# qfall/tools

Measured on AMD Instinct MI355X. Metric: preimages/sec (whole node) + HBM-BW% for samp_p, n=512 q~2^30 batch=4096, higher is better.
Workload: dtype f64+int64

## Files before the change

tools_amd/csrc/psf_kernels.hpp:

```cpp
#pragma once
#include <hip/hip_runtime.h>
#include <cstdint>
#include "psf_rng.hpp"

namespace psf {

typedef double d4 __attribute__((ext_vector_type(4)));
typedef int v4i __attribute__((ext_vector_type(4)));
typedef __attribute__((address_space(3))) void* lds_void_ptr;

constexpr int TR_BM = 128;
constexpr int TR_BN = 128;
#ifndef PSF_TR_BK
#define PSF_TR_BK 16
#endif
constexpr int TR_BK = PSF_TR_BK;
constexpr int TR_CHUNK = TR_BM * TR_BK;
constexpr int TR_KB_PER_BLOCK = TR_BM / TR_BK;

__host__ __device__ inline size_t tr_rowblock_base(size_t bi) { return (size_t)TR_KB_PER_BLOCK * bi * (bi + 1) / 2; }
__host__ __device__ inline size_t tr_total_chunks(size_t nbi) { return (size_t)TR_KB_PER_BLOCK * nbi * (nbi + 1) / 2; }

__host__ __device__ inline int tr_chunk_pos(int r, int kk) {
  return ((kk >> 2) * 8 + (r >> 4)) * 64 + ((kk & 3) << 4) + (r & 15);
}

template <bool PACKED>
__global__ void k_repack_L(const double* __restrict__ src, size_t ld, size_t m, double* __restrict__ dst, size_t nbi) {
  const size_t total = tr_total_chunks(nbi) * TR_CHUNK;
  for (size_t g = (size_t)blockIdx.x * blockDim.x + threadIdx.x; g < total; g += (size_t)gridDim.x * blockDim.x) {
    const size_t chunk = g / TR_CHUNK;
    const int pos = (int)(g % TR_CHUNK);
    size_t bi = (size_t)((sqrt(1.0 + 8.0 * (double)chunk / TR_KB_PER_BLOCK) - 1.0) * 0.5);
    while (tr_rowblock_base(bi + 1) <= chunk) ++bi;
    while (tr_rowblock_base(bi) > chunk) --bi;
    const size_t bk = chunk - tr_rowblock_base(bi);
    const int ks = pos >> 9, tile = (pos >> 6) & 7, lane = pos & 63;
    const size_t row = bi * TR_BM + tile * 16 + (lane & 15);
    const size_t col = bk * TR_BK + ks * 4 + (lane >> 4);
    double v = 0.0;
    if (row < m && col <= row) v = PACKED ? src[row * (row + 1) / 2 + col] : src[row * ld + col];
    dst[g] = v;
  }
}

__global__ void k_unpack_L(const double* __restrict__ chunks, size_t first, size_t total, double* __restrict__ packed) {
  for (size_t g0 = (size_t)blockIdx.x * blockDim.x + threadIdx.x; g0 < total; g0 += (size_t)gridDim.x * blockDim.x) {
    const size_t g = first + g0;
    size_t row = (size_t)((sqrt(1.0 + 8.0 * (double)g) - 1.0) * 0.5);
    while ((row + 1) * (row + 2) / 2 <= g) ++row;
    while (row * (row + 1) / 2 > g) --row;
    const size_t col = g - row * (row + 1) / 2;
    const size_t bi = row / TR_BM, bk = col / TR_BK;
    const size_t chunk = tr_rowblock_base(bi) + bk;
    packed[g0] = chunks[chunk * TR_CHUNK + tr_chunk_pos((int)(row % TR_BM), (int)(col % TR_BK))];
  }
}

constexpr int NR_SEG = 4096;
__host__ inline uint32_t nr_segment(size_t total) {
  size_t seg = (total / 4096 + 63) / 64 * 64;
  if (seg < 128) seg = 128;
  return (uint32_t)(seg > (size_t)NR_SEG ? (size_t)NR_SEG : seg);
}
__device__ inline int lane_rank(uint64_t mask);
__host__ __device__ inline uint32_t udiv_magic_of(uint32_t d) { return d < 2 ? 0u : (uint32_t)((((uint64_t)1 << 32) + d - 1) / d); }
__device__ inline void udivmod_magic(uint32_t o, uint32_t d, uint32_t M, uint32_t* q, uint32_t* r) {
  const uint32_t qq = M ? __umulhi(o, M) : o;
  *q = qq;
  *r = o - qq * d;
}

struct NormalsFixed { size_t split; int8_t* planes; size_t plane_bytes; size_t ld; double* X; double h; };
constexpr int kFixPlanes = 5;

__global__ __launch_bounds__(256) void k_normals_wave(uint64_t seed, uint64_t first_index, size_t m, size_t B, size_t nkb, size_t nbj,
                                                      double* __restrict__ Dt, int* __restrict__ fail, NormalsFixed fx, uint32_t ncf, uint32_t seg) {
  const int lane = threadIdx.x & 63;
  const size_t total = ncf >= 0x100u ? nkb * 4 * 4 * (size_t)(ncf - 0x100u) : ncf ? nkb * 4 * (size_t)ncf * 64 : nbj * nkb * TR_CHUNK;
  const size_t seg0 = ((size_t)blockIdx.x * 4 + (threadIdx.x >> 6)) * seg;
  if (seg0 >= total) return;
  const size_t seg1 = seg0 + seg < total ? seg0 + seg : total;
  const size_t chunk0 = seg0 / TR_CHUNK;
  constexpr int NCH = NR_SEG / TR_CHUNK + 1;
  size_t cbj[NCH], cbk[NCH];
// ... 41 lines not shown
        const uint64_t index = first_index + b;
        const U4 w = philox(seed, (uint32_t)coord, (uint32_t)index, t, tag_word(TAG_NORMAL, index));
        const double u = (double)(((((uint64_t)w.y << 32) | w.x) >> 11) + 1) * 0x1.0p-53;
        const uint64_t vv = (((uint64_t)w.w << 32) | w.z) >> 12;
        const double x = (((double)(2 * vv + 1) * 0x1.0p-52 - 1.0) * 0.8577638849607068) / u;
        {
          const float xf = (float)x, uf = (float)u;
          const float e32 = __builtin_amdgcn_exp2f(-0.36067376f * (xf * xf));
          const bool sure = uf <= e32 * 0.9998f, never = uf > e32 * 1.0002f;
          accept = sure;
          if (!sure && !never) accept = u <= det_exp(-0.25 * (x * x));
        }
        v = x;
        if (!accept && ++t >= kMaxAttempts) { accept = true; f = 1; v = 0.0; }
        if (accept && fx.planes && coord >= fx.split) {
          const double sc = floor(v * 0x1.0p32 + 0.5);
          if (!(fabs(sc) < 0x1.0p38)) f = 1;
          long long qv = (long long)sc;
          v = sc * 0x1.0p-32;
          const size_t c = coord - fx.split;
          const size_t addr = ((c >> 4) * fx.ld + b) * 16 + (c & 15);
#pragma unroll
          for (int pl = 0; pl < kFixPlanes; ++pl) {
            const long long dg = (long long)(int8_t)(qv & 0xff);
            fx.planes[(size_t)pl * fx.plane_bytes + addr] = (int8_t)dg;
            qv = (qv - dg) >> 8;
          }
          fx.X[coord * fx.ld + b] = fx.h * v;
        }
      }
      if (accept) Dt[my] = v;
    }
    const uint64_t mask = __ballot(accept);
    if (mask) {
      const size_t nid = next_free + (size_t)lane_rank(mask);
      if (accept) {
        my = nid;
        active = nid < seg1;
        t = 0;
        if (active) locate(nid, &coord, &b);
      }
      next_free += (size_t)__popcll(mask);
    }
  }
  if (f) atomicOr(fail, 1);
}

__global__ __launch_bounds__(256) void k_narrow_rows(const int64_t* __restrict__ src, int32_t* __restrict__ dst, size_t count, int* __restrict__ overflow) {
  const size_t stride = (size_t)gridDim.x * 256;
  int bad = 0;
  const size_t pairs = count / 2;
  for (size_t i = (size_t)blockIdx.x * 256 + threadIdx.x; i < pairs; i += stride) {
    const longlong2 v = reinterpret_cast<const longlong2*>(src)[i];
    bad |= (v.x != (int64_t)(int32_t)v.x) | (v.y != (int64_t)(int32_t)v.y);
    reinterpret_cast<int2*>(dst)[i] = make_int2((int32_t)v.x, (int32_t)v.y);
  }
  if ((count & 1) && blockIdx.x == 0 && threadIdx.x == 0) {
    const int64_t v = src[count - 1];
    bad |= v != (int64_t)(int32_t)v;
    dst[count - 1] = (int32_t)v;
  }
  if (bad) atomicOr(overflow, 1);
}

__global__ __launch_bounds__(256) void k_copy_words(const uint64_t* __restrict__ host_src, uint64_t* __restrict__ dst, size_t count) {
  const size_t stride = (size_t)gridDim.x * 256, pairs = count / 2;
  typedef unsigned long long u2 __attribute__((ext_vector_type(2)));
  for (size_t i = (size_t)blockIdx.x * 256 + threadIdx.x; i < pairs; i += stride)
    reinterpret_cast<u2*>(dst)[i] = __builtin_nontemporal_load(reinterpret_cast<const u2*>(host_src) + i);
  if ((count & 1) && blockIdx.x == 0 && threadIdx.x == 0) dst[count - 1] = host_src[count - 1];
}

__global__ void k_export_normals(const double* __restrict__ Dt, size_t m, size_t B, size_t nkb, double* __restrict__ out , uint32_t ncf) {
  const size_t total = m * B;
  for (size_t g = (size_t)blockIdx.x * blockDim.x + threadIdx.x; g < total; g += (size_t)gridDim.x * blockDim.x) {
    const size_t b = g / m, coord = g % m;
    if (ncf >= 0x100u) { out[g] = Dt[((coord / 4) * (ncf - 0x100u) + b) * 4 + coord % 4]; continue; }
    if (ncf) { out[g] = Dt[((coord / 4) * ncf + b / 16) * 64 + (coord % 4) * 16 + b % 16]; continue; }
    const size_t chunk = (b / TR_BN) * nkb + coord / TR_BK;
    out[g] = Dt[chunk * TR_CHUNK + tr_chunk_pos((int)(b % TR_BN), (int)(coord % TR_BK))];
  }
}

__device__ inline void tr_map_block(unsigned id, int nbi, int nbj, int GR, int GC, int* bi, int* bj) {
  const int ncg = (nbj + GC - 1) / GC, nrg = (nbi + GR - 1) / GR;
  const unsigned xcd = id & 7u, slot = id >> 3;
  const unsigned group = (slot / (GR * GC)) * 8u + xcd;
  const unsigned t = slot % (GR * GC);
  const int rg = nrg - 1 - (int)(group / ncg), cg = (int)(group % ncg);
  *bi = rg * GR + (GR - 1 - (int)(t / GC));
  *bj = cg * GC + (int)(t % GC);
  if (rg < 0) *bi = -1;
}
__host__ inline unsigned tr_grid_size(int nbi, int nbj, int GR = 8, int GC = 8) {
  const int ncg = (nbj + GC - 1) / GC, nrg = (nbi + GR - 1) / GR;
  const unsigned groups = (unsigned)(ncg * nrg);
  const unsigned rounds = (groups + 7) / 8;
  return rounds * 8u * (unsigned)(GR * GC);
}

#ifdef TRMM_CLOCK_PROBE
__device__ unsigned long long g_trmm_clk[4];
__device__ unsigned long long* g_trmm_log;
#define TR_CLK_BEGIN const unsigned long long clk0 = clock64(), rt0 = wall_clock64();
#define TR_CLK_END if (threadIdx.x == 0) { const unsigned long long rt1 = wall_clock64(); atomicAdd(&g_trmm_clk[0], clock64() - clk0); atomicAdd(&g_trmm_clk[1], rt1 - rt0); atomicAdd(&g_trmm_clk[2], 1ull); \
    if (g_trmm_log) { g_trmm_log[2 * (size_t)blockIdx.x] = rt0; g_trmm_log[2 * (size_t)blockIdx.x + 1] = rt1; } }
#else
#define TR_CLK_BEGIN
#define TR_CLK_END
#endif

constexpr int TR_PD = 6;
#define TR_LOAD8(dst, voff, base, imm) asm volatile("global_load_dwordx2 %0, %1, %2 offset:" #imm : "=v"(dst) : "v"(voff), "s"(base) : "memory")
#define TR_WAIT(n, A, Bv) asm volatile("s_waitcnt vmcnt(" #n ")" : "+v"(A[0]), "+v"(A[1]), "+v"(A[2]), "+v"(A[3]), "+v"(Bv[0]), "+v"(Bv[1]), "+v"(Bv[2]), "+v"(Bv[3]))

constexpr int TR_BIG_PD = 4;
#ifndef TR_BIG_UNROLL
#define TR_BIG_UNROLL 2
#endif
#define TR_WAIT12(n, A, Bv) asm volatile("s_waitcnt vmcnt(" #n ")" : "+v"(A[0]), "+v"(A[1]), "+v"(A[2]), "+v"(A[3]), "+v"(A[4]), "+v"(A[5]), "+v"(A[6]), "+v"(A[7]), \
                                         "+v"(Bv[0]), "+v"(Bv[1]), "+v"(Bv[2]), "+v"(Bv[3]))
__global__ __launch_bounds__(256, 1) void k_trmm_f64_big(const double* __restrict__ Lt, const double* __restrict__ Dt,
                                                         double* __restrict__ X, int nbi, int nbj, size_t nkb, size_t ldx, int GR, int GC, size_t row_hi) {
  int bt, bj;
  const int nbt = (nbi + 1) / 2;
  tr_map_block(blockIdx.x, nbt, nbj, GR, GC, &bt, &bj);
  if (bt < 0 || bt >= nbt || bj >= nbj) return;
  TR_CLK_BEGIN
  const int tid = threadIdx.x, lane = tid & 63;
  const int wave = __builtin_amdgcn_readfirstlane(tid >> 6);
  const int wr = wave >> 1, wc = wave & 1;
  const int bi = 2 * bt + wr;
  if (bi < nbi) {
    const int nsteps = TR_KB_PER_BLOCK * (bi + 1) * (TR_BK / 4);
    const double* gA = Lt + tr_rowblock_base((size_t)bi) * TR_CHUNK;
    const double* gB = Dt + (size_t)bj * nkb * TR_CHUNK + (size_t)(wc * 4) * 64;
    const uint32_t voff = (uint32_t)lane * 8u;
    d4 acc[8][4];
#pragma unroll
    for (int i = 0; i < 8; ++i)
#pragma unroll
      for (int j = 0; j < 4; ++j) acc[i][j] = d4{0.0, 0.0, 0.0, 0.0};
    double a[TR_BIG_PD][8], b[TR_BIG_PD][4];
    auto issue = [&](double (&av)[8], double (&bv)[4], int s) {
      const double* pa = gA + (size_t)s * 512;
      const double* pb = gB + (size_t)s * 512;
      TR_LOAD8(av[0], voff, pa, 0); TR_LOAD8(av[1], voff, pa, 512); TR_LOAD8(av[2], voff, pa, 1024); TR_LOAD8(av[3], voff, pa, 1536);
      TR_LOAD8(av[4], voff, pa, 2048); TR_LOAD8(av[5], voff, pa, 2560); TR_LOAD8(av[6], voff, pa, 3072); TR_LOAD8(av[7], voff, pa, 3584);
      TR_LOAD8(bv[0], voff, pb, 0); TR_LOAD8(bv[1], voff, pb, 512); TR_LOAD8(bv[2], voff, pb, 1024); TR_LOAD8(bv[3], voff, pb, 1536);
    };
#define TR_MFMA(i, j) asm volatile("v_mfma_f64_16x16x4_f64 %0, %1, %2, %0" : "+a"(acc[i][j]) : "v"(av[i]), "v"(bv[j]))
    auto step = [&](double (&av)[8], double (&bv)[4], int sn) {
      const double* pa = gA + (size_t)sn * 512;
      const double* pb = gB + (size_t)sn * 512;
      TR_MFMA(0, 0); TR_MFMA(0, 1); TR_MFMA(0, 2); TR_MFMA(0, 3); TR_LOAD8(av[0], voff, pa, 0);
      TR_MFMA(1, 0); TR_MFMA(1, 1); TR_MFMA(1, 2); TR_MFMA(1, 3); TR_LOAD8(av[1], voff, pa, 512);
      TR_MFMA(2, 0); TR_MFMA(2, 1); TR_MFMA(2, 2); TR_MFMA(2, 3); TR_LOAD8(av[2], voff, pa, 1024);
      TR_MFMA(3, 0); TR_MFMA(3, 1); TR_MFMA(3, 2); TR_MFMA(3, 3); TR_LOAD8(av[3], voff, pa, 1536);
      TR_MFMA(4, 0); TR_MFMA(4, 1); TR_MFMA(4, 2); TR_MFMA(4, 3); TR_LOAD8(av[4], voff, pa, 2048);
      TR_MFMA(5, 0); TR_MFMA(5, 1); TR_MFMA(5, 2); TR_MFMA(5, 3); TR_LOAD8(av[5], voff, pa, 2560);
      TR_MFMA(6, 3); TR_MFMA(7, 3); TR_LOAD8(bv[3], voff, pb, 1536);
      TR_MFMA(6, 2); TR_MFMA(7, 2); TR_LOAD8(bv[2], voff, pb, 1024);
      TR_MFMA(6, 1); TR_MFMA(7, 1); TR_LOAD8(bv[1], voff, pb, 512);
      TR_MFMA(6, 0); TR_MFMA(7, 0); TR_LOAD8(bv[0], voff, pb, 0);
      TR_LOAD8(av[6], voff, pa, 3072); TR_LOAD8(av[7], voff, pa, 3584);
    };
#pragma unroll
    for (int u = 0; u < TR_BIG_PD; ++u) issue(a[u], b[u], u);
    for (int s0 = 0; s0 < nsteps; s0 += TR_BIG_PD * TR_BIG_UNROLL) {
#pragma unroll
      for (int rnd = 0; rnd < TR_BIG_UNROLL; ++rnd)
#pragma unroll
      for (int u = 0; u < TR_BIG_PD; ++u) {
        TR_WAIT12(36, a[u], b[u]);
        static_assert(TR_BIG_PD == 4, "the wait count above is 12 (TR_BIG_PD - 1)");
        int sn = s0 + rnd * TR_BIG_PD + u + TR_BIG_PD;
        sn = sn < nsteps ? sn : nsteps - 1;
        step(a[u], b[u], sn);
      }
    }
#undef TR_MFMA
#pragma unroll
    for (int u = 0; u < TR_BIG_PD; ++u) TR_WAIT12(0, a[u], b[u]);
    asm volatile("s_nop 15\n\ts_nop 15\n\ts_nop 15\n\ts_nop 15\n\ts_nop 15" ::: "memory");
    const size_t row0 = (size_t)bi * TR_BM, col0 = (size_t)bj * TR_BN + wc * 64;
#pragma unroll
    for (int i = 0; i < 8; ++i)
#pragma unroll
      for (int j = 0; j < 4; ++j)
#pragma unroll
        for (int r = 0; r < 4; ++r)
        {
          const size_t row = row0 + i * 16 + (lane >> 4) + 4 * r;
          if (row < row_hi) X[row * ldx + col0 + j * 16 + (lane & 15)] = acc[i][j][r];
        }
  }
  TR_CLK_END
}

constexpr int PR_SEG = 4096;
constexpr long long kDigitRangeP = (1ll << 23) - 1;

__device__ inline double wave_xor_sum(double x) {
  typedef unsigned int u2v __attribute__((ext_vector_type(2)));
  auto mk = [](uint32_t lo, uint32_t hi) { return __hiloint2double((int)hi, (int)lo); };
  uint32_t lo = (uint32_t)__double2loint(x), hi = (uint32_t)__double2hiint(x);
  { const u2v a = __builtin_amdgcn_permlane32_swap(lo, lo, false, false), b = __builtin_amdgcn_permlane32_swap(hi, hi, false, false);
    x = mk(a.x, b.x) + mk(a.y, b.y); lo = (uint32_t)__double2loint(x); hi = (uint32_t)__double2hiint(x); }
  { const u2v a = __builtin_amdgcn_permlane16_swap(lo, lo, false, false), b = __builtin_amdgcn_permlane16_swap(hi, hi, false, false);
    x = mk(a.x, b.x) + mk(a.y, b.y); lo = (uint32_t)__double2loint(x); hi = (uint32_t)__double2hiint(x); }
  { const int pl = __builtin_amdgcn_update_dpp(0, (int)lo, 0x128, 0xf, 0xf, false), ph = __builtin_amdgcn_update_dpp(0, (int)hi, 0x128, 0xf, 0xf, false);
    x = x + mk((uint32_t)pl, (uint32_t)ph); lo = (uint32_t)__double2loint(x); hi = (uint32_t)__double2hiint(x); }
  { int pl = __builtin_amdgcn_update_dpp(0, (int)lo, 0x104, 0xf, 0x5, false); pl = __builtin_amdgcn_update_dpp(pl, (int)lo, 0x114, 0xf, 0xa, false);
    int ph = __builtin_amdgcn_update_dpp(0, (int)hi, 0x104, 0xf, 0x5, false); ph = __builtin_amdgcn_update_dpp(ph, (int)hi, 0x114, 0xf, 0xa, false);
    x = x + mk((uint32_t)pl, (uint32_t)ph); lo = (uint32_t)__double2loint(x); hi = (uint32_t)__double2hiint(x); }
  { const int pl = __builtin_amdgcn_update_dpp(0, (int)lo, 0x4e, 0xf, 0xf, false), ph = __builtin_amdgcn_update_dpp(0, (int)hi, 0x4e, 0xf, 0xf, false);
    x = x + mk((uint32_t)pl, (uint32_t)ph); lo = (uint32_t)__double2loint(x); hi = (uint32_t)__double2hiint(x); }
  { const int pl = __builtin_amdgcn_update_dpp(0, (int)lo, 0xb1, 0xf, 0xf, false), ph = __builtin_amdgcn_update_dpp(0, (int)hi, 0xb1, 0xf, 0xf, false);
    x = x + mk((uint32_t)pl, (uint32_t)ph); }
  return x;
}

__device__ inline int lane_rank(uint64_t mask) {
  return (int)__builtin_amdgcn_mbcnt_hi((uint32_t)(mask >> 32), __builtin_amdgcn_mbcnt_lo((uint32_t)mask, 0));
}

__global__ __launch_bounds__(256) void k_perturb_round_wave(uint64_t seed, uint64_t first_index, size_t m, size_t B, size_t ld,
                                                            const double* __restrict__ X, SampleZParams sp, int32_t* __restrict__ P,
                                                            int* __restrict__ fail) {
  const int lane = threadIdx.x & 63;
  const size_t wave_id = (size_t)blockIdx.x * 4 + (threadIdx.x >> 6);
  const size_t total = m * B;
  const size_t seg0 = wave_id * PR_SEG;
  if (seg0 >= total) return;
  const size_t seg1 = seg0 + PR_SEG < total ? seg0 + PR_SEG : total;
  const size_t coord0 = seg0 / B;
  const uint32_t b00 = (uint32_t)(seg0 % B), B32 = (uint32_t)B;
  const bool one_wrap = B32 >= (uint32_t)PR_SEG;
  auto locate = [&](size_t g, size_t* coord, uint32_t* bb) {
    const uint32_t o = b00 + (uint32_t)(g - seg0);
    if (one_wrap) {
      const bool wrap = o >= B32;
      *coord = coord0 + (wrap ? 1 : 0);
      *bb = wrap ? o - B32 : o;
    } else {
      *coord = coord0 + o / B32;
      *bb = o % B32;
    }
  };
  auto centre_of = [&](size_t g) -> double {
    if (g >= seg1) return 0.0;
    size_t cc; uint32_t bb;
    locate(g, &cc, &bb);
    return X[cc * ld + bb];
  };
  size_t base = seg0 + 64;
  double w0 = centre_of(base + lane), w1 = centre_of(base + 64 + lane), w2 = centre_of(base + 128 + lane);
  size_t my = seg0 + lane, next_free = seg0 + 64;
  bool active = my < seg1;
  double c = centre_of(my);
  size_t coord = 0; uint32_t b = 0;
  locate(active ? my : seg0, &coord, &b);
  uint32_t t = 0;
  int f = 0;
  while (__ballot(active)) {
    bool accept = false;
    long long x = 0;
    if (active) {
      const uint64_t index = first_index + b;
      const uint32_t tw = tag_word(TAG_PERTURB, index);
      const SzRange rg = sz_range(c, sp);
      accept = sz_group4(seed, (uint32_t)coord, (uint32_t)index, tw, t, rg, c, sp.inv_s, &x);
      if (!accept && ++t >= kMaxAttempts / 4) { accept = true; f = 1; x = (long long)floor(c + 0.5); }
      if (accept) {
        if (x > kDigitRangeP || x < -kDigitRangeP) f = 1;
        P[coord * ld + b] = (int32_t)x;
      }
    }
    const uint64_t mask = __ballot(accept);
    if (mask) {
      const size_t nid = next_free + (size_t)lane_rank(mask);
// ... 1448 lines not shown
```

tools_amd/csrc/psfp.hip:

```cpp
#include <hip/hip_runtime.h>
#include <cmath>
#include <cstdio>
#include <cstdlib>
#include <cstring>
#include <chrono>
#include <string>
#include <thread>
#include <atomic>
#include <mutex>
#include <functional>
#include <vector>
#include "../../include/psf_mi355x.h"
#include "psf_host.hpp"
#include "psf_kernels.hpp"
#include "psf_stream_kernels.hpp"
#include "psf_gpv_kernels.hpp"
#include "psf_np_kernels.hpp"
#include "psf_chol_kernels.hpp"
#include "psf_gemm_kernels.hpp"
#include "psf_sdma.hpp"
#include "psf_ntt_api.hpp"

struct KeygenClock {
  bool on; const char* what; std::chrono::steady_clock::time_point t0, last;
// ... 951 lines not shown
    const size_t cw = std::min(round_up(ncols, 64), ld);
    hipLaunchKernelGGL(k_split_P, dim3(grid_for(h->K_pad / 16 * cw, 256, 256 * 64)), dim3(256), 0, st, P, h->m, ld, h->K_pad / 16, P8, h->dFail, (size_t)0, cw);
    const dim3 grid((unsigned)((ncols + 63) / 64), (unsigned)(h->n_pad / 64), (unsigned)z.splits);
    auto fp = [&](auto k_tt, auto k_tf, auto k_ft, auto k_ff) { return z.fold128 ? (z.pow2 ? k_tt : k_tf) : (z.pow2 ? k_ft : k_ff); };
#define ZQM(NA_) case NA_: hipLaunchKernelGGL(fp(k_zq_mfma<NA_, true, true>, k_zq_mfma<NA_, true, false>, k_zq_mfma<NA_, false, true>, k_zq_mfma<NA_, false, false>), grid, dim3(256), \
                                              2 * (NA_ + 3) * 4096, st, h->dA8, h->n_pad, h->K_pad, P8, ld, z.ks, h->zc, (int)h->wide, h->dPart, (size_t)0, h->dFail); break;
    switch (h->NA) { ZQM(1) ZQM(2) ZQM(3) ZQM(4) ZQM(5) ZQM(6) ZQM(7) ZQM(8) default: break; }
#undef ZQM
  } else {
    const dim3 grid((unsigned)z.splits, (unsigned)((h->n + 15) / 16));
    if (z.form == ZqPlan::SMALL32)
      hipLaunchKernelGGL(by_cols(ncols, k_syndrome_small32<1>, k_syndrome_small32<2>, k_syndrome_small32<4>), grid, dim3(512), 0, st, h->dA32, h->n, h->m, P, ld, ncols, h->q, 16,
                         h->dPart, h->n_pad, (size_t)0);
    else
      hipLaunchKernelGGL(by_cols(ncols, k_syndrome_small<1>, k_syndrome_small<2>, k_syndrome_small<4>), grid, dim3(512), 0, st, h->dA, h->n, h->m, P, ld, ncols, h->q, 16,
                         h->dPart, h->n_pad, (size_t)0);
  }
  hipLaunchKernelGGL(z.wave_combine ? k_zq_combine_wave<false> : k_zq_combine, dim3(z.wave_combine ? (unsigned)((h->n * ncols + 3) / 4) : grid_for(h->n * ncols, 256, 256 * 32)),
                     dim3(256), 0, st, mode, h->dPart, z.splits, h->n, h->n_pad, ld, ncols, h->q, U, out, ldo, (size_t)0);
}

struct SampPlan {
  bool one_launch = false;
  int bc = 0; uint32_t ncf = 0, nseg = 0; size_t nwaves = 0;
  enum Product : uint8_t { TASKS, TILES64, TILES32, TILES96, BIG } product = BIG;
  int RT = 2, NB = 1, ncg = 1;
  bool compact = false; int GR = 8, GC = 4;
  bool tail = false; int tail_ntask = 0, tail_rt = 2;
  enum Round : uint8_t { ROUND_TAB, ROUND_TAB_ROW, ROUND_LEAN, ROUND_WAVE } round = ROUND_WAVE;
  uint32_t seg = 0; size_t rwaves = 0;
  ZqPlan syn;
  enum Gadget : uint8_t { G_WAVE, G_ROW, G_QUAD, G_QUEUE, G_LOCKSTEP } gadget = G_LOCKSTEP;
  bool k32 = false; int gq_p = 0;
  enum Recombine : uint8_t { R_SMALL, R_SMALL2, R_WG, R_TILES } recombine = R_TILES;
  size_t rc_lds = 0; unsigned rc_wgs = 0; int nbf = 0;
  bool rc_big = false; int rsplits = 1, kps = 0;
  bool small_copies = false, r8 = false;
};

struct BatchDims { size_t nbj; int zq_split_cap; };

static SampPlan plan_samp_p(const psfp_handle* h, size_t B, const BatchDims* bd = nullptr) {
  SampPlan p;
  const size_t m = h->m;
  const size_t nbj = bd ? bd->nbj : h->nbj;
  size_t fused_max = 64;
  if (const char* e = psf_exp_env("PSF_FUSED_MAX")) fused_max = (size_t)std::atol(e);
  p.one_launch = !h->structured && !h->no_slice && h->gadget_queue && m <= (size_t)FS_MAX_M && h->n <= 64 && B <= fused_max;
  if (p.one_launch) return p;
  bool stream = B <= 1472 || (B >= 1537 && B <= 1728) || (h->mL < 16384 && B <= 2048);
  if (const char* e = psf_exp_env("PSF_TRMM_STREAM_MAX")) stream = B <= std::min<size_t>((size_t)std::atol(e), 2048);
  const char* shape = psf_exp_env("PSF_TRMM_STREAM_SHAPE");
  p.NB = B <= 16 ? 1 : B <= 64 ? 2 : 4;
  size_t wg_min = 33;
  if (const char* e = psf_exp_env("PSF_STREAM_WG")) wg_min = std::atol(e) > 0 ? (size_t)std::atol(e) : (size_t)-1;
  size_t wg_max = 64;
  if (const char* e = psf_exp_env("PSF_STREAM_WG_MAX")) wg_max = std::min<size_t>((size_t)std::atol(e), 64);
  const bool small_factor = h->mL < 16384;
  bool wg192 = stream && ((B > 128 && B <= 960 && (((B + 63) / 64) & 1) != 0) || B > 1088 || (small_factor && B > 64)) && !shape;
  if (const char* e = psf_exp_env("PSF_STREAM_WG192")) {
    long lo = 0, hi = 0;
    wg192 = std::sscanf(e, "%ld:%ld", &lo, &hi) == 2 && lo >= 65 && hi <= 2048 && stream && B >= (size_t)lo && B <= (size_t)hi && !shape;
  }
  const bool wg = stream && ((B >= wg_min && B <= wg_max) || wg192) && !shape;
  const char* e32 = psf_exp_env("PSF_STREAM_WG32");
  const bool wg32 = stream && !wg && B >= 17 && B <= 32 && !shape && !(e32 && std::atoi(e32) == 0);
  const char* e96 = psf_exp_env("PSF_STREAM_WG96");
  const bool wg96 = stream && !wg && !small_factor && B >= 65 && B <= 96 && !shape && !(e96 && std::atoi(e96) == 0);
  if (wg) p.NB = 4;
  if (wg32 || wg96) p.NB = 2;
  if (shape) std::sscanf(shape, "%d,%d", &p.RT, &p.NB);
  if (!(p.NB == 1 || p.NB == 2 || p.NB == 4 || p.NB == 8)) p.NB = 1;
  p.ncg = (int)((B + 16 * (size_t)p.NB - 1) / (16 * (size_t)p.NB));
  const char* ecd = psf_exp_env("PSF_COMPACT_D");
  p.compact = stream && !h->structured && !(ecd && std::atoi(ecd) == 0);
  if (p.compact && p.NB == 1 && p.ncg == 1 && !(ecd && std::atoi(ecd) == 1)) { p.bc = 1; while ((size_t)p.bc < B) p.bc <<= 1; }
  p.ncf = p.bc ? 0x100u + (uint32_t)p.bc : p.compact ? (uint32_t)(p.ncg * p.NB) : 0u;
  const size_t npos = p.bc ? h->nkb * 4 * 4 * (size_t)p.bc : p.ncf ? h->nkb * 4 * (size_t)p.ncf * 64 : nbj * h->nkb * TR_CHUNK;
  p.nseg = nr_segment(npos);
  if (const char* e = psf_exp_env("PSF_NR_SEG")) { const long v = std::atol(e); if (v >= 64 && v <= NR_SEG && v % 64 == 0) p.nseg = (uint32_t)v; }
  p.nwaves = (npos + p.nseg - 1) / p.nseg;
  if (!stream) {
    p.product = SampPlan::BIG;
    if (B < 4096 || nbj % 4 != 0) { p.GR = 16; p.GC = 2; }
    if (const char* e1 = psf_exp_env("PSF_TRMM_GR")) if (const char* e2 = psf_exp_env("PSF_TRMM_GC")) { p.GR = std::atoi(e1); p.GC = std::atoi(e2); }
    if (p.GR < 1 || p.GC < 1 || p.GR * p.GC != 32) { p.GR = 8; p.GC = 4; }
  } else p.product = wg96 ? SampPlan::TILES96 : wg32 ? SampPlan::TILES32 : wg ? SampPlan::TILES64 : SampPlan::TASKS;
  if (stream && p.bc && B <= 2 && p.RT == 2 && p.NB == 1 && !h->structured && h->szR.sh == 16 && !(h->prm.flags & PSFP_FLAG_NO_PERTURB)) {
    p.small_copies = true;
    const char* fe = psf_exp_env("PSF_FUSED_TAIL");
    if (h->dA32T && small_usable(h) && !(fe && std::atoi(fe) == 0)) {
      if (const char* e = psf_exp_env("PSF_FUSED_RT")) p.tail_rt = std::atoi(e) == 1 ? 1 : 2;
      p.tail_ntask = ((int)((h->mL + 15) / 16) + p.tail_rt - 1) / p.tail_rt;
      p.tail = true;
    }
  }
  p.r8 = h->structured;
  const char* renv = psf_exp_env("PSF_ROUND");
  if (h->szR.sh == 16 && !(renv && !std::strcmp(renv, "wave"))) {
    p.seg = prl_segment(m * B);
    if (const char* e = psf_exp_env("PSF_PRL_SEG")) { const long v = std::atol(e); if (v >= 64 && v <= PRL_SEG && v % 64 == 0) p.seg = (uint32_t)v; }
    p.round = SampPlan::ROUND_LEAN;
    if (h->szF && !(renv && !std::strcmp(renv, "lean"))) {
      if (B % 64 == 0 && B >= 1024 && B <= (size_t)PRL_SEG && (size_t)p.seg > B) p.seg = (uint32_t)B;
      p.round = (size_t)p.seg == B ? SampPlan::ROUND_TAB_ROW : SampPlan::ROUND_TAB;
    }
    p.rwaves = (m * B + p.seg - 1) / p.seg;
  } else p.rwaves = (m * B + PR_SEG - 1) / PR_SEG;
  p.syn = plan_zq(h, B, true, bd ? bd->zq_split_cap : -1);
  p.small_copies |= p.syn.form != ZqPlan::MFMA;
  const size_t nB = h->n * B;
  const char* genv = psf_exp_env("PSF_GADGET_WAVE");
  const size_t wave_max = genv ? (size_t)std::atol(genv) : 2048;
  const char* genvq = psf_exp_env("PSF_GADGET_QUAD");
  const size_t quad_max = genvq ? (size_t)std::atol(genvq) : 98304;
  const char* genvr = psf_exp_env("PSF_GADGET_ROW");
  const size_t row_max = genvr ? (size_t)std::atol(genvr) : 10240;
  p.k32 = h->k <= 32;
  if (!h->gadget_queue) p.gadget = SampPlan::G_LOCKSTEP;
  else if (nB <= wave_max) p.gadget = SampPlan::G_WAVE;
  else if (nB <= row_max && h->k <= 64) p.gadget = SampPlan::G_ROW;
  else if (nB <= quad_max && h->k <= 64) p.gadget = SampPlan::G_QUAD;
  else {
    p.gadget = SampPlan::G_QUEUE;
    p.gq_p = gq_problems_for((uint32_t)h->k, nB);
    if (const char* e = psf_exp_env("PSF_GQ_P")) { const int v = std::atoi(e); if (v >= 1 && v <= 128 && (v & (v - 1)) == 0) p.gq_p = v; }
  }
  size_t small_max = 4;
  if (const char* e = psf_exp_env("PSF_RECOMBINE_SMALL")) small_max = std::min<size_t>((size_t)std::atol(e), 4);
  p.rc_lds = 32 * (h->ldr / 16) * B;
  size_t rs_max = 448;
  if (const char* e = psf_exp_env("PSF_RECOMBINE_STREAM")) rs_max = (size_t)std::min<long>(std::atol(e), 1024);
  if (B <= small_max && p.rc_lds <= 150 * 1024) {
    p.recombine = h->small_state == 2 ? SampPlan::R_SMALL2 : SampPlan::R_SMALL;
    p.rc_wgs = (unsigned)std::min<size_t>((h->mb + 7) / 8, p.rc_lds > 64 * 1024 ? 256 : 512);
    p.small_copies = true;
  } else if (B <= rs_max && h->ldr % 128 == 0 && h->mb >= 64) {
    p.recombine = SampPlan::R_WG;
    p.nbf = B > 64 ? 4 : (int)((B + 15) / 16);
  } else {
    p.recombine = SampPlan::R_TILES;
    p.rc_big = (B % 256 == 0 || B > rs_max) && h->mb >= 512 && (h->ldr / 64) % 2 == 0;
    p.r8 = p.r8 || p.rc_big;
    const unsigned tiles = (unsigned)((B + 127) / 128) * (unsigned)((h->mb + 127) / 128);
    const int nks = (int)(h->ldr / 64);
    p.kps = nks;
    if (!p.rc_big && tiles < 1024 && nks >= 16) {
      const int splits = (int)(2048 / tiles);
      p.kps = std::max((nks + splits - 1) / splits, 8);
      p.kps += p.kps & 1;
      p.rsplits = (nks + p.kps - 1) / p.kps;
    }
  }
  return p;
}

static_assert(SampPlan::BIG == PSFP_PRODUCT_BIG && SampPlan::TILES96 == PSFP_PRODUCT_TILES96 && SampPlan::TILES64 == PSFP_PRODUCT_TILES64 && SampPlan::ROUND_WAVE == PSFP_ROUND_WAVE &&
              SampPlan::ROUND_TAB_ROW == PSFP_ROUND_TAB_ROW && ZqPlan::MFMA == PSFP_ZQ_MFMA && ZqPlan::SMALL32 == PSFP_ZQ_SMALL32 && SampPlan::G_LOCKSTEP == PSFP_GADGET_LOCKSTEP &&
              SampPlan::G_QUAD == PSFP_GADGET_QUAD && SampPlan::R_TILES == PSFP_RECOMBINE_TILES && SampPlan::R_SMALL2 == PSFP_RECOMBINE_SMALL2 && PSFP_PLAN_RSPLITS == 22,
              "the enumerators of include/psf_mi355x.h follow SampPlan");
static void plan_fields(const SampPlan& p, int* f) {
  const int v[PSFP_PLAN_FIELDS] = {p.one_launch, p.product, p.RT, p.NB, p.ncg, p.bc, p.compact, p.GR, p.GC, p.tail, p.round, p.syn.form, p.syn.splits, p.syn.fold128, p.syn.pow2,
                                   p.syn.wave_combine, p.gadget, p.k32, p.gq_p, p.recombine, p.nbf, p.rc_big, p.rsplits};
  std::memcpy(f, v, sizeof(v));
}

static void prepare_samp_p(psfp_handle* h, hipStream_t st, SampPlan& p) {
  if (p.small_copies) ensure_small_copies(h, st);
  if (p.tail) {
    const size_t need = (size_t)p.tail_ntask * h->n * 2;
    if (need > h->partF_cap) {
      hipFree(h->dPartF); h->dPartF = nullptr; h->partF_cap = 0;
      if (hipMalloc(&h->dPartF, need * sizeof(uint64_t)) == hipSuccess) h->partF_cap = need; else (void)hipGetLastError();
    }
    p.tail = h->dPartF != nullptr;
  }
  if (p.r8) ensure_R8(h, st);
}

static void normals_stage(psfp_handle* h, hipStream_t st, const SampPlan& p, uint64_t seed, uint64_t first_index, size_t B) {
  ScopedTimer t(h, st, "k_normals");
  const NormalsFixed fx = h->structured ? NormalsFixed{h->mb, h->dD8, h->ldr * h->ld, h->ld, h->dX, h->h_const} : NormalsFixed{0, nullptr, 0, 0, nullptr, 0.0};
  hipLaunchKernelGGL(k_normals_wave, dim3((unsigned)((p.nwaves + 3) / 4)), dim3(256), 0, st, seed, first_index, h->m, B, h->nkb, h->nbj, h->dDt, h->dFail, fx, p.ncf, p.nseg);
}

static void product_stage(psfp_handle* h, hipStream_t st, const SampPlan& p, size_t B) {
  ScopedTimer t(h, st, "k_trmm_f64");
  const size_t row_hi = h->structured ? h->mb : h->M_pad;
  if (p.product == SampPlan::BIG) {
    hipLaunchKernelGGL(k_trmm_f64_big, dim3(tr_grid_size(((int)h->nbiL + 1) / 2, (int)h->nbj, p.GR, p.GC)), dim3(256), 0, st, h->dLt, h->dDt, h->dX, (int)h->nbiL, (int)h->nbj,
                       h->nkb, h->ld, p.GR, p.GC, row_hi);
    return;
  }
  auto geom = [&](int rt, int ncg, int bc) { StreamGeom g; g.ntile = ((int)((h->mL + 15) / 16) + rt - 1) / rt; g.ncg = ncg; g.ntask = g.ntile * ncg; g.bc = bc; return g; };
  auto go = [&](auto kern, const StreamGeom& g, unsigned grid, unsigned block, size_t lds) { hipLaunchKernelGGL(kern, dim3(grid), dim3(block), lds, st, h->dLt, h->dDt, h->dX, g, h->nkb, h->ld, row_hi); };
  auto cd = [&](auto k0, auto k1) { return p.compact ? k1 : k0; };
  const auto wg64 = cd(k_trmm_stream_wg<TSW64_H, TSW64_NBUF, 0, 2>, k_trmm_stream_wg<TSW64_H, TSW64_NBUF, 1, 2>);
  const auto wg32 = cd(k_trmm_stream_wg32<TSW_H, TSW_NBUF, 0>, k_trmm_stream_wg32<TSW_H, TSW_NBUF, 1>);
  StreamGeom g = geom(4, p.product == SampPlan::TILES96 ? 1 : p.ncg, 0);
  const unsigned nwg = (unsigned)((g.ntask + 1) / 2);
  if (p.product == SampPlan::TILES96) {
    g.ncf = 6;
    go(wg64, g, nwg, 512, TSW_LDS);
    g.cf_base = 4;
    go(wg32, g, nwg, 512, TSW32_LDS);
  } else if (p.product == SampPlan::TILES32) go(wg32, g, nwg, 512, TSW32_LDS);
  else if (p.product == SampPlan::TILES64) go(wg64, g, p.ncg > 1 ? 8 * ((nwg + 7) / 8) : nwg, 512, TSW_LDS);
  else {
    auto ts = [&](auto kern, int rt, int half) { const StreamGeom gt = geom(rt, p.ncg, p.bc); go(kern, gt, (unsigned)((gt.ntask + 2 * half - 1) / (2 * half)), 128 * half, 0); };
#define TS_GO(rt, nb, pd, half) ts(cd(k_trmm_stream<rt, nb, pd, half, 0>, k_trmm_stream<rt, nb, pd, half, 1>), rt, half)
    if (p.bc && p.RT == 2 && p.NB == 1) ts(k_trmm_stream<2, 1, 12, 2, 2>, 2, 2);
    else if (p.bc && p.NB == 1) ts(k_trmm_stream<1, 1, 8, 4, 2>, 1, 4);
    else if (p.RT == 2 && p.NB == 1) TS_GO(2, 1, 12, 2);
    else if (p.RT == 2 && p.NB == 2 && B <= 32) TS_GO(2, 2, 8, 2);
    else if (p.RT == 2 && p.NB == 2) TS_GO(2, 2, 16, 4);
    else if (p.RT == 2 && p.NB == 4) TS_GO(2, 4, 8, 4);
    else if (p.RT == 4 && p.NB == 2) TS_GO(4, 2, 10, 4);
    else if (p.RT == 1 && p.NB == 8) TS_GO(1, 8, 8, 4);
    else if (p.RT == 1 && p.NB == 4) TS_GO(1, 4, 8, 4);
    else if (p.RT == 1 && p.NB == 2) TS_GO(1, 2, 8, 4);
    else TS_GO(1, 1, 8, 4);
#undef TS_GO
  }
}

static void round_stage(psfp_handle* h, hipStream_t st, const SampPlan& p, uint64_t seed, uint64_t first_index, size_t B) {
  const size_t ld = h->ld, m = h->m;
  if (p.tail) {
    ScopedTimer t(h, st, "k_round+A p");
    StreamGeom g;
    g.ntile = p.tail_ntask; g.ncg = 1; g.ntask = p.tail_ntask; g.bc = p.bc;
    const StreamFuse fz{seed, first_index, m, h->szR, h->dP, ld, h->dA32T, h->n, h->q, h->dPartF, h->dFail};
    hipLaunchKernelGGL(p.tail_rt == 1 ? k_round_syndrome_small<1> : k_round_syndrome_small<2>, dim3((unsigned)((g.ntask + 3) / 4)), dim3(256), 0, st, h->dX, ld,
                       h->structured ? h->mb : h->M_pad, g, fz);
    return;
  }
  ScopedTimer t(h, st, "k_perturb_round");
  const dim3 grid((unsigned)((p.rwaves + 3) / 4));
  switch (p.round) {
    case SampPlan::ROUND_TAB:
    case SampPlan::ROUND_TAB_ROW:
      hipLaunchKernelGGL(p.round == SampPlan::ROUND_TAB_ROW ? k_perturb_round_tab<true> : k_perturb_round_tab<false>, grid, dim3(256), (size_t)h->szR.n_int * h->szF * sizeof(uint32_t),
                         st, seed, first_index, m, B, ld, h->dX, h->szR, h->dP, h->dFail, p.seg, SzTable{h->dSzTab, h->szF, h->szR.n_int});
      break;
    case SampPlan::ROUND_LEAN:
      hipLaunchKernelGGL(k_perturb_round_lean, grid, dim3(256), 0, st, seed, first_index, m, B, ld, h->dX, h->szR, h->dP, h->dFail, p.seg);
      break;
    case SampPlan::ROUND_WAVE:
      hipLaunchKernelGGL(k_perturb_round_wave, grid, dim3(256), 0, st, seed, first_index, m, B, ld, h->dX, h->szR, h->dP, h->dFail);
      break;
  }
}

static void syndrome_stage(psfp_handle* h, hipStream_t st, const SampPlan& p, size_t B, const uint64_t* d_u) {
  ScopedTimer t(h, st, "k_zq_matmul(syndrome)");
  if (p.tail)
    hipLaunchKernelGGL((k_zq_combine_wave<true>), dim3((unsigned)((h->n * B + 3) / 4)), dim3(256), 0, st, ZQ_SYNDROME, h->dPartF, p.tail_ntask, h->n, h->n, (size_t)p.bc, B, h->q, d_u, h->dV, h->ld, (size_t)0);
  else launch_zq(h, st, p.syn, ZQ_SYNDROME, h->dP, h->dP8, B, d_u, h->dV, h->ld);
}

static void gadget_stage(psfp_handle* h, hipStream_t st, const SampPlan& p, uint64_t seed, uint64_t first_index, size_t B) {
  const size_t ld = h->ld, nB = h->n * B;
  ScopedTimer t(h, st, "k_gadget");
  const GadgetTablesQ tq{h->dSk, h->dGso, h->dNorm2, h->dSz, h->dRng};
  auto go = [&](auto kern, dim3 grid, size_t lds, auto tables, auto... extra) {
    hipLaunchKernelGGL(kern, grid, dim3(256), lds, st, seed, first_index, (uint32_t)h->n, (uint32_t)h->k, h->q, h->prm.gp.base, B, ld, h->dV, tables, h->dZlo, h->dZhi, h->dFail, extra...);
  };
  switch (p.gadget) {
    case SampPlan::G_WAVE: go(k_gadget_wave, dim3((unsigned)((nB + 3) / 4)), 0, tq); break;
    case SampPlan::G_ROW: go(p.k32 ? k_gadget_quad<2, 16> : k_gadget_quad<4, 16>, dim3((unsigned)((nB + 15) / 16)), 0, tq); break;
    case SampPlan::G_QUAD: go(p.k32 ? k_gadget_quad<8> : k_gadget_quad<16>, dim3((unsigned)((nB + 63) / 64)), 0, tq); break;
    case SampPlan::G_QUEUE:
      go(p.gq_p == 128 ? k_gadget_queue<true> : k_gadget_queue<false>, dim3((unsigned)((nB + (size_t)GQ_WAVES * p.gq_p - 1) / ((size_t)GQ_WAVES * p.gq_p))),
         gadget_queue_lds_bytes(h->k, p.gq_p), tq, p.gq_p);
// ... 705 lines not shown
```

Baseline: 69980.

## Remap big TRMM waves to row-block quarters and skip zero diagonal fragments

Each workgroup's four waves now share one row block and cover four 64-column quarters, where they previously split across two row blocks and two column halves. Waves in a group therefore see equal work and reuse the same L fragments. The last diagonal chunk of k-steps is peeled into a compile-time-unrolled tail that skips MFMAs and loads for fragments that are zero in the lower-triangular block. Accumulators move to fixed AGPRs with inline-asm init and direct AGPR stores. The tile-group heuristic changes too, with GC forced even, and the hand-counted waitcnt values and AGPR clobbers could break if register allocation differs.

```diff
diff --git a/tools_amd/csrc/psf_kernels.hpp b/tools_amd/csrc/psf_kernels.hpp
--- a/tools_amd/csrc/psf_kernels.hpp
+++ b/tools_amd/csrc/psf_kernels.hpp
@@ -1,6 +1,7 @@
 #pragma once
 #include <hip/hip_runtime.h>
 #include <cstdint>
+#include <utility>
 #include "psf_rng.hpp"
 
 namespace psf {
@@ -208,7 +209,7 @@
   }
 }
 
-__device__ inline void tr_map_block(unsigned id, int nbi, int nbj, int GR, int GC, int* bi, int* bj) {
+__host__ __device__ inline void tr_map_block(unsigned id, int nbi, int nbj, int GR, int GC, int* bi, int* bj) {
   const int ncg = (nbj + GC - 1) / GC, nrg = (nbi + GR - 1) / GR;
   const unsigned xcd = id & 7u, slot = id >> 3;
   const unsigned group = (slot / (GR * GC)) * 8u + xcd;
@@ -246,27 +247,54 @@
 #endif
 #define TR_WAIT12(n, A, Bv) asm volatile("s_waitcnt vmcnt(" #n ")" : "+v"(A[0]), "+v"(A[1]), "+v"(A[2]), "+v"(A[3]), "+v"(A[4]), "+v"(A[5]), "+v"(A[6]), "+v"(A[7]), \
                                          "+v"(Bv[0]), "+v"(Bv[1]), "+v"(Bv[2]), "+v"(Bv[3]))
-__global__ __launch_bounds__(256, 1) void k_trmm_f64_big(const double* __restrict__ Lt, const double* __restrict__ Dt,
-                                                         double* __restrict__ X, int nbi, int nbj, size_t nkb, size_t ldx, int GR, int GC, size_t row_hi) {
+constexpr int TR_DIAG_STEPS = TR_KB_PER_BLOCK * (TR_BK / 4);
+__host__ __device__ constexpr int tr_diag_first_frag(int t) { return t / 4; }
+__host__ __device__ constexpr int tr_diag_loads(int t) { return t >= TR_DIAG_STEPS ? 0 : 12 - tr_diag_first_frag(t); }
+template <int T> struct TrStep { static constexpr int value = T; };
+template <class F, int... Is> __device__ __forceinline__ void tr_for_steps(F&& f, std::integer_sequence<int, Is...>) { (f(TrStep<Is>{}), ...); }
+#define TR_A10(p) "a" #p "0", "a" #p "1", "a" #p "2", "a" #p "3", "a" #p "4", "a" #p "5", "a" #p "6", "a" #p "7", "a" #p "8", "a" #p "9"
+#define TR_A100(p) TR_A10(p##0), TR_A10(p##1), TR_A10(p##2), TR_A10(p##3), TR_A10(p##4), TR_A10(p##5), TR_A10(p##6), TR_A10(p##7), TR_A10(p##8), TR_A10(p##9)
+#define TR_ACC_CLOBBERS TR_A10(), TR_A10(1), TR_A10(2), TR_A10(3), TR_A10(4), TR_A10(5), TR_A10(6), TR_A10(7), TR_A10(8), TR_A10(9), TR_A100(1), \
+                        TR_A10(20), TR_A10(21), TR_A10(22), TR_A10(23), TR_A10(24), "a250", "a251", "a252", "a253", "a254", "a255"
+
+__host__ inline unsigned tr_big_grid_size(int nbi, int nbj, int GR, int GC) { return tr_grid_size(nbi, (nbj + 1) / 2, 2 * GR, GC / 2); }
+__host__ __device__ inline bool tr_big_map(unsigned id, int wave, int nbi, int nbj, int GR, int GC, int* bi, int* quarter) {
+  int bp;
+  tr_map_block(id, nbi, (nbj + 1) / 2, 2 * GR, GC / 2, bi, &bp);
+  *quarter = 4 * bp + wave;
+  return *bi >= 0 && *bi < nbi && (*quarter >> 1) < nbj;
+}
+#ifdef PSF_EXPERIMENTS
+__host__ inline unsigned tr_pairs_grid_size(int nbi, int nbj, int GR, int GC) { return tr_grid_size((nbi + 1) / 2, nbj, GR, GC); }
+__host__ __device__ inline bool tr_pairs_map(unsigned id, int wave, int nbi, int nbj, int GR, int GC, int* bi, int* quarter) {
   int bt, bj;
-  const int nbt = (nbi + 1) / 2;
-  tr_map_block(blockIdx.x, nbt, nbj, GR, GC, &bt, &bj);
-  if (bt < 0 || bt >= nbt || bj >= nbj) return;
-  TR_CLK_BEGIN
+  tr_map_block(id, (nbi + 1) / 2, nbj, GR, GC, &bt, &bj);
+  *bi = 2 * bt + (wave >> 1);
+  *quarter = 2 * bj + (wave & 1);
+  return bt >= 0 && *bi < nbi && bj < nbj;
+}
+#endif
+
+template <bool PAIRS, bool DIAG>
+__device__ __forceinline__ void tr_big_body(const double* __restrict__ Lt, const double* __restrict__ Dt, double* __restrict__ X, int nbi, int nbj, size_t nkb, size_t ldx,
+                                            int GR, int GC, size_t row_hi) {
   const int tid = threadIdx.x, lane = tid & 63;
   const int wave = __builtin_amdgcn_readfirstlane(tid >> 6);
-  const int wr = wave >> 1, wc = wave & 1;
-  const int bi = 2 * bt + wr;
-  if (bi < nbi) {
+  int bi, quarter;
+  bool work;
+#ifdef PSF_EXPERIMENTS
+  if (PAIRS) work = tr_pairs_map(blockIdx.x, wave, nbi, nbj, GR, GC, &bi, &quarter); else
+#endif
+  work = tr_big_map(blockIdx.x, wave, nbi, nbj, GR, GC, &bi, &quarter);
+  if (!work) return;
+  {
     const int nsteps = TR_KB_PER_BLOCK * (bi + 1) * (TR_BK / 4);
+    const bool diag = DIAG && bi > 0;
+    const int nloop = diag ? nsteps - TR_DIAG_STEPS : nsteps;
     const double* gA = Lt + tr_rowblock_base((size_t)bi) * TR_CHUNK;
-    const double* gB = Dt + (size_t)bj * nkb * TR_CHUNK + (size_t)(wc * 4) * 64;
+    const double* gB = Dt + (size_t)(quarter >> 1) * nkb * TR_CHUNK + (size_t)((quarter & 1) * 4) * 64;
     const uint32_t voff = (uint32_t)lane * 8u;
-    d4 acc[8][4];
-#pragma unroll
-    for (int i = 0; i < 8; ++i)
-#pragma unroll
-      for (int j = 0; j < 4; ++j) acc[i][j] = d4{0.0, 0.0, 0.0, 0.0};
+    asm volatile(".set .Ltr_acc, 0\n\t.rept 256\n\tv_accvgpr_write_b32 a[.Ltr_acc], 0\n\t.set .Ltr_acc, .Ltr_acc + 1\n\t.endr" ::: TR_ACC_CLOBBERS);
     double a[TR_BIG_PD][8], b[TR_BIG_PD][4];
     auto issue = [&](double (&av)[8], double (&bv)[4], int s) {
       const double* pa = gA + (size_t)s * 512;
@@ -275,7 +303,7 @@
       TR_LOAD8(av[4], voff, pa, 2048); TR_LOAD8(av[5], voff, pa, 2560); TR_LOAD8(av[6], voff, pa, 3072); TR_LOAD8(av[7], voff, pa, 3584);
       TR_LOAD8(bv[0], voff, pb, 0); TR_LOAD8(bv[1], voff, pb, 512); TR_LOAD8(bv[2], voff, pb, 1024); TR_LOAD8(bv[3], voff, pb, 1536);
     };
-#define TR_MFMA(i, j) asm volatile("v_mfma_f64_16x16x4_f64 %0, %1, %2, %0" : "+a"(acc[i][j]) : "v"(av[i]), "v"(bv[j]))
+#define TR_MFMA(i, j) asm volatile("v_mfma_f64_16x16x4_f64 a[%2:%3], %0, %1, a[%2:%3]" : : "v"(av[i]), "v"(bv[j]), "n"(8 * (4 * (i) + (j))), "n"(8 * (4 * (i) + (j)) + 7))
     auto step = [&](double (&av)[8], double (&bv)[4], int sn) {
       const double* pa = gA + (size_t)sn * 512;
       const double* pb = gB + (size_t)sn * 512;
@@ -293,7 +321,8 @@
     };
 #pragma unroll
     for (int u = 0; u < TR_BIG_PD; ++u) issue(a[u], b[u], u);
-    for (int s0 = 0; s0 < nsteps; s0 += TR_BIG_PD * TR_BIG_UNROLL) {
+    int s0 = 0;
+    do {
 #pragma unroll
       for (int rnd = 0; rnd < TR_BIG_UNROLL; ++rnd)
 #pragma unroll
@@ -304,25 +333,70 @@
         sn = sn < nsteps ? sn : nsteps - 1;
         step(a[u], b[u], sn);
       }
+      s0 += TR_BIG_PD * TR_BIG_UNROLL;
+    } while (s0 < nloop);
+    if (diag) {
+      static_assert(TR_BIG_PD == 4 && TR_DIAG_STEPS == 32 && TR_DIAG_STEPS % TR_BIG_PD == 0, "the ring slot of k-step t is t % 4 in the loop and here");
+      const double* gAd = gA + (size_t)nloop * 512;
+      const double* gBd = gB + (size_t)nloop * 512;
+#define TR_DMFMA(i, j) do { if constexpr (i >= i0) TR_MFMA(i, j); } while (0)
+#define TR_DLOAD_A(i, imm) do { if constexpr (tn < TR_DIAG_STEPS && i >= in0) TR_LOAD8(av[i], voff, pa, imm); } while (0)
+#define TR_DLOAD_B(j, imm) do { if constexpr (tn < TR_DIAG_STEPS) TR_LOAD8(bv[j], voff, pb, imm); } while (0)
+      auto dstep = [&](auto tc) {
+        constexpr int t = decltype(tc)::value, tn = t + TR_BIG_PD;
+        constexpr int i0 = tr_diag_first_frag(t), in0 = tr_diag_first_frag(tn);
+        constexpr int in_flight = tr_diag_loads(t + 1) + tr_diag_loads(t + 2) + tr_diag_loads(t + 3);
+        double (&av)[8] = a[t % TR_BIG_PD];
+        double (&bv)[4] = b[t % TR_BIG_PD];
+        const double* pa = gAd + (size_t)tn * 512;
+        const double* pb = gBd + (size_t)tn * 512;
+        asm volatile("s_waitcnt vmcnt(%12)" : "+v"(av[0]), "+v"(av[1]), "+v"(av[2]), "+v"(av[3]), "+v"(av[4]), "+v"(av[5]), "+v"(av[6]), "+v"(av[7]),
+                     "+v"(bv[0]), "+v"(bv[1]), "+v"(bv[2]), "+v"(bv[3]) : "n"(in_flight));
+        TR_DMFMA(0, 0); TR_DMFMA(0, 1); TR_DMFMA(0, 2); TR_DMFMA(0, 3); TR_DLOAD_A(0, 0);
+        TR_DMFMA(1, 0); TR_DMFMA(1, 1); TR_DMFMA(1, 2); TR_DMFMA(1, 3); TR_DLOAD_A(1, 512);
+        TR_DMFMA(2, 0); TR_DMFMA(2, 1); TR_DMFMA(2, 2); TR_DMFMA(2, 3); TR_DLOAD_A(2, 1024);
+        TR_DMFMA(3, 0); TR_DMFMA(3, 1); TR_DMFMA(3, 2); TR_DMFMA(3, 3); TR_DLOAD_A(3, 1536);
+        TR_DMFMA(4, 0); TR_DMFMA(4, 1); TR_DMFMA(4, 2); TR_DMFMA(4, 3); TR_DLOAD_A(4, 2048);
+        TR_DMFMA(5, 0); TR_DMFMA(5, 1); TR_DMFMA(5, 2); TR_DMFMA(5, 3); TR_DLOAD_A(5, 2560);
+        TR_DMFMA(6, 3); TR_DMFMA(7, 3); TR_DLOAD_B(3, 1536);
+        TR_DMFMA(6, 2); TR_DMFMA(7, 2); TR_DLOAD_B(2, 1024);
+        TR_DMFMA(6, 1); TR_DMFMA(7, 1); TR_DLOAD_B(1, 512);
+        TR_DMFMA(6, 0); TR_DMFMA(7, 0); TR_DLOAD_B(0, 0);
+        TR_DLOAD_A(6, 3072); TR_DLOAD_A(7, 3584);
+      };
+      tr_for_steps(dstep, std::make_integer_sequence<int, TR_DIAG_STEPS>{});
+#undef TR_DLOAD_B
+#undef TR_DLOAD_A
+#undef TR_DMFMA
     }
 #undef TR_MFMA
 #pragma unroll
     for (int u = 0; u < TR_BIG_PD; ++u) TR_WAIT12(0, a[u], b[u]);
     asm volatile("s_nop 15\n\ts_nop 15\n\ts_nop 15\n\ts_nop 15\n\ts_nop 15" ::: "memory");
-    const size_t row0 = (size_t)bi * TR_BM, col0 = (size_t)bj * TR_BN + wc * 64;
-#pragma unroll
-    for (int i = 0; i < 8; ++i)
-#pragma unroll
-      for (int j = 0; j < 4; ++j)
-#pragma unroll
-        for (int r = 0; r < 4; ++r)
-        {
-          const size_t row = row0 + i * 16 + (lane >> 4) + 4 * r;
-          if (row < row_hi) X[row * ldx + col0 + j * 16 + (lane & 15)] = acc[i][j][r];
-        }
-  }
+    const size_t row0 = (size_t)bi * TR_BM + (lane >> 4), col0 = (size_t)quarter * 64 + (lane & 15);
+    auto store = [&](auto ec) {
+      constexpr int e = decltype(ec)::value, i = e >> 4, j = (e >> 2) & 3, r = e & 3;
+      const size_t row = row0 + i * 16 + 4 * r;
+      double* px = X + row * ldx + col0 + j * 16;
+      if (row < row_hi) asm volatile("global_store_dwordx2 %0, a[%1:%2], off" : : "v"(px), "n"(8 * (4 * i + j) + 2 * r), "n"(8 * (4 * i + j) + 2 * r + 1) : "memory");
+    };
+    tr_for_steps(store, std::make_integer_sequence<int, 128>{});
+  }
+}
+
+__global__ __launch_bounds__(256, 1) void k_trmm_f64_big(const double* __restrict__ Lt, const double* __restrict__ Dt,
+                                                         double* __restrict__ X, int nbi, int nbj, size_t nkb, size_t ldx, int GR, int GC, size_t row_hi) {
+  TR_CLK_BEGIN
+  tr_big_body<false, true>(Lt, Dt, X, nbi, nbj, nkb, ldx, GR, GC, row_hi);
   TR_CLK_END
 }
+#ifdef PSF_EXPERIMENTS
+template <bool PAIRS, bool DIAG>
+__global__ __launch_bounds__(256, 1) void k_trmm_f64_big_arm(const double* __restrict__ Lt, const double* __restrict__ Dt,
+                                                             double* __restrict__ X, int nbi, int nbj, size_t nkb, size_t ldx, int GR, int GC, size_t row_hi) {
+  tr_big_body<PAIRS, DIAG>(Lt, Dt, X, nbi, nbj, nkb, ldx, GR, GC, row_hi);
+}
+#endif
 
 constexpr int PR_SEG = 4096;
 constexpr long long kDigitRangeP = (1ll << 23) - 1;
diff --git a/tools_amd/csrc/psfp.hip b/tools_amd/csrc/psfp.hip
--- a/tools_amd/csrc/psfp.hip
+++ b/tools_amd/csrc/psfp.hip
@@ -1057,9 +1057,9 @@
   p.nwaves = (npos + p.nseg - 1) / p.nseg;
   if (!stream) {
     p.product = SampPlan::BIG;
-    if (B < 4096 || nbj % 4 != 0) { p.GR = 16; p.GC = 2; }
+    if (nbj % 4 != 0 || nbj < 28) { p.GR = 16; p.GC = 2; }
     if (const char* e1 = psf_exp_env("PSF_TRMM_GR")) if (const char* e2 = psf_exp_env("PSF_TRMM_GC")) { p.GR = std::atoi(e1); p.GC = std::atoi(e2); }
-    if (p.GR < 1 || p.GC < 1 || p.GR * p.GC != 32) { p.GR = 8; p.GC = 4; }
+    if (p.GR < 1 || p.GC < 2 || p.GC % 2 != 0 || p.GR * p.GC != 32) { p.GR = 8; p.GC = 4; }
   } else p.product = wg96 ? SampPlan::TILES96 : wg32 ? SampPlan::TILES32 : wg ? SampPlan::TILES64 : SampPlan::TASKS;
   if (stream && p.bc && B <= 2 && p.RT == 2 && p.NB == 1 && !h->structured && h->szR.sh == 16 && !(h->prm.flags & PSFP_FLAG_NO_PERTURB)) {
     p.small_copies = true;
@@ -1163,8 +1163,16 @@
   ScopedTimer t(h, st, "k_trmm_f64");
   const size_t row_hi = h->structured ? h->mb : h->M_pad;
   if (p.product == SampPlan::BIG) {
-    hipLaunchKernelGGL(k_trmm_f64_big, dim3(tr_grid_size(((int)h->nbiL + 1) / 2, (int)h->nbj, p.GR, p.GC)), dim3(256), 0, st, h->dLt, h->dDt, h->dX, (int)h->nbiL, (int)h->nbj,
-                       h->nkb, h->ld, p.GR, p.GC, row_hi);
+    const int nbi = (int)h->nbiL, nbj = (int)h->nbj;
+#ifdef PSF_EXPERIMENTS
+    if (const char* e = psf_exp_env("PSF_TRMM_FORM")) {
+      auto arm = [&](auto kern, unsigned grid) { hipLaunchKernelGGL(kern, dim3(grid), dim3(256), 0, st, h->dLt, h->dDt, h->dX, nbi, nbj, h->nkb, h->ld, p.GR, p.GC, row_hi); };
+      if (!std::strcmp(e, "pairs")) { arm(k_trmm_f64_big_arm<true, false>, tr_pairs_grid_size(nbi, nbj, p.GR, p.GC)); return; }
+      if (!std::strcmp(e, "pairs_diag")) { arm(k_trmm_f64_big_arm<true, true>, tr_pairs_grid_size(nbi, nbj, p.GR, p.GC)); return; }
+      if (!std::strcmp(e, "quarters")) { arm(k_trmm_f64_big_arm<false, false>, tr_big_grid_size(nbi, nbj, p.GR, p.GC)); return; }
+    }
+#endif
+    hipLaunchKernelGGL(k_trmm_f64_big, dim3(tr_big_grid_size(nbi, nbj, p.GR, p.GC)), dim3(256), 0, st, h->dLt, h->dDt, h->dX, nbi, nbj, h->nkb, h->ld, p.GR, p.GC, row_hi);
     return;
   }
   auto geom = [&](int rt, int ncg, int bc) { StreamGeom g; g.ntile = ((int)((h->mL + 15) / 16) + rt - 1) / rt; g.ncg = ncg; g.ntask = g.ntile * ncg; g.bc = bc; return g; };
```

Measured after the change: 70610, median of 6. Within noise of the previous version (+0.9%).
